# ZhengdiYu/Arbitrary-Hands-3D-Reconstruction

Measured on AMD Instinct MI355X. Metric: frames/sec (2-hand mesh) at 512x512 batch-64; vertex L2 vs ref, higher is better.
Workload: dtype f32; 1 GPU; configs[2]: synthetic 512x512 RGB batch=64 per GPU, HRNet-W32 backbone, fp32; frames_per_gpu=64, global_batch=64, parallelism=frame-sharded x1, gather=none (one rank), contexts_in_turn=2

## Files before the change

### arbitrary-hands-3d-reconstruction_amd/csrc/acrmi.hip

```cpp
#include "acrmi_ctx.h"
#include "score_plan.h"
#include "surface_contact_plan.h"
#include "vertex_color_plan.h"

#include <initializer_list>
#include <type_traits>

std::string g_err;

int fail(acrmi_ctx* c, int code, const char* fmt, ...) {
  char buf[512];
  va_list ap;
  va_start(ap, fmt);
  vsnprintf(buf, sizeof buf, fmt, ap);
  va_end(ap);
  if (c) c->err = buf; else g_err = buf;
  return code;
}

void release_weights(acrmi_ctx* c) {
  if (c->weights_ref && c->weights_ref->fetch_sub(1) == 1) {
    (void)hipFree(c->weights);
    delete c->weights_ref;
  }
// ... 1062 lines not shown
  if (!c->faces_topo[0] || !c->faces_topo[1]) return fail(c, ACRMI_ESTATE, "%s: MANO faces not loaded (acrmi_load_faces)", who);
  ON_DEVICE(c);
  RenderScratch sc;
  if (int r = render_scratch(c, n, &sc)) return r;
  hipError_t e = launch_render_region_prep(slots, offsets, region_frame, n, n_frames, H, W, ACRMI_SLOT, ACRMI_SLOT_FLAG,
                                           colors_host ? colors_host : kHandColors, sc.mesh_frame, sc.mesh_topo, sc.rgb, sc.view,
                                           (hipStream_t)stream);
  if (e != hipSuccess) return fail(c, ACRMI_EHIP, "render region prep: %s", hipGetErrorString(e));
  e = render_launch(c, sc, verts, cam_trans, nullptr, sc.view, focal, visible_weight, img_in, img_out, ids_out, 2 * n, n_frames, H, W,
                    (hipStream_t)stream, vcol);
  return e == hipSuccess ? ACRMI_OK : fail(c, ACRMI_EHIP, "render regions: %s", hipGetErrorString(e));
}

int acrmi_render_regions(acrmi_ctx* c, const float* verts, const float* cam_trans, const float* slots, int n, const float* offsets,
                         const int32_t* region_frame, const float* colors_host, float focal, float visible_weight,
                         const uint8_t* img_in, uint8_t* img_out, int n_frames, int H, int W, int32_t* ids_out, void* stream) {
  return render_regions_call(c, "acrmi_render_regions", false, nullptr, verts, cam_trans, slots, n, offsets, region_frame, colors_host,
                             focal, visible_weight, img_in, img_out, n_frames, H, W, ids_out, stream);
}

int acrmi_render_regions_colored(acrmi_ctx* c, const float* verts, const float* cam_trans, const float* slots, int n,
                                 const float* offsets, const int32_t* region_frame, const float* colors_host, const float* vcol,
                                 float focal, float visible_weight, const uint8_t* img_in, uint8_t* img_out, int n_frames, int H,
                                 int W, int32_t* ids_out, void* stream) {
  return render_regions_call(c, "acrmi_render_regions_colored", true, vcol, verts, cam_trans, slots, n, offsets, region_frame,
                             colors_host, focal, visible_weight, img_in, img_out, n_frames, H, W, ids_out, stream);
}

int acrmi_overlay_regions(acrmi_ctx* c, int what, const float* slots, const float* pj2d_org, int n, const float* offsets,
                          const int32_t* region_frame, int bgr, const uint8_t* img_in, uint8_t* out, uint8_t* out2, int n_frames,
                          int H, int W, void* stream) {
  if (!offsets || !region_frame || n > 0x3fffffff) return fail(c, ACRMI_EINVAL, "acrmi_overlay_regions: bad arguments");
  if (int r = check_overlay(c, "acrmi_overlay_regions", what, slots, pj2d_org, n, img_in, out, out2, n_frames, H, W)) return r;
  ON_DEVICE(c);
  hipError_t e;
  if (what == ACRMI_OVERLAY_SKELETON) {
    if (n > c->region_hand_cap) {
      if (c->region_hand_frame) {
        HIPCHK(c, hipDeviceSynchronize());
        (void)hipFree(c->region_hand_frame);
        c->region_hand_frame = nullptr;
        c->region_hand_cap = 0;
      }
      HIPCHK(c, hipMalloc(&c->region_hand_frame, sizeof(int32_t) * 2 * (size_t)n));
      c->region_hand_cap = n;
    }
    e = launch_render_region_prep(slots, offsets, region_frame, n, n_frames, H, W, ACRMI_SLOT, ACRMI_SLOT_FLAG, nullptr,
                                  c->region_hand_frame, nullptr, nullptr, nullptr, (hipStream_t)stream);
    if (e != hipSuccess) return fail(c, ACRMI_EHIP, "overlay region prep: %s", hipGetErrorString(e));
    e = skeleton_launch(pj2d_org, nullptr, c->region_hand_frame, 0, 2 * n, n_frames, H, W, bgr, img_in, out, (hipStream_t)stream);
  } else {
    RegionHeatmapArgs a{};
    if (int r = heatmap_fill(c, "acrmi_overlay_regions", a, n, offsets, bgr, img_in, out, out2, H, W)) return r;
    a.n_frames = n_frames; a.region_frame = region_frame;
    e = launch_region_heatmap(a, (hipStream_t)stream);
  }
  return e == hipSuccess ? ACRMI_OK : fail(c, ACRMI_EHIP, "overlay regions: %s", hipGetErrorString(e));
}

int acrmi_stream_create(int device, void** stream) {
  if (!stream) return fail(nullptr, ACRMI_EINVAL, "acrmi_stream_create: null argument");
  int prev = 0;
  if (hipGetDevice(&prev) != hipSuccess || hipSetDevice(device) != hipSuccess)
    return fail(nullptr, ACRMI_EHIP, "acrmi_stream_create: cannot select device %d", device);
  hipStream_t st = nullptr;
  const hipError_t e = hipStreamCreateWithFlags(&st, hipStreamNonBlocking);
  (void)hipSetDevice(prev);
  if (e != hipSuccess) return fail(nullptr, ACRMI_EHIP, "hipStreamCreate: %s", hipGetErrorString(e));
  *stream = st;
  return ACRMI_OK;
}

int acrmi_stream_destroy(void* stream) {
  if (!stream) return ACRMI_OK;
  const hipError_t e = hipStreamDestroy((hipStream_t)stream);
  return e == hipSuccess ? ACRMI_OK : fail(nullptr, ACRMI_EHIP, "hipStreamDestroy: %s", hipGetErrorString(e));
}

int acrmi_tune(int key, int value) {
  if (key == 0) { conv_force_cfg(value); return ACRMI_OK; }
  if (key == 3) { conv_set_phase_delay(value); return ACRMI_OK; }
  if (key == 4) { conv_set_xcd_swizzle(value); return ACRMI_OK; }
  if (key == 5) { program_set_grouping(value != 0); return ACRMI_OK; }
  static long long* dbg = nullptr;
  if (key == 1) {
    if (value && !dbg) { if (hipMalloc(&dbg, 128 * sizeof(long long)) != hipSuccess) return ACRMI_EHIP; }
    if (dbg) (void)hipMemset(dbg, 0, 128 * sizeof(long long));
    conv_set_debug(value ? dbg : nullptr);
    return ACRMI_OK;
  }
  if (key == 2) {
    if (!dbg) return ACRMI_OK;
    long long h[128];
    if (hipDeviceSynchronize() != hipSuccess) return ACRMI_EHIP;
    if (hipMemcpy(h, dbg, sizeof h, hipMemcpyDeviceToHost) != hipSuccess) return ACRMI_EHIP;
    const int n = (int)h[63];
    printf("conv stamps (%d):", n);
    for (int i = 1; i < n && i < 60; ++i) printf(" %lld", h[i] - h[i - 1]);
    printf("\n");
    const int nl = (int)h[127];
    if (nl > 0) {
      printf("loader stamps (%d):", nl);
      for (int i = 1; i < nl && i < 60; ++i) printf(" %lld", h[64 + i] - h[64 + i - 1]);
      printf("\n");
    }
    return ACRMI_OK;
  }
  return fail(nullptr, ACRMI_EINVAL, "acrmi_tune: unknown key %d", key);
}

}
```

### arbitrary-hands-3d-reconstruction_amd/csrc/conv_mfma.hip

```cpp
#include "conv_frame.h"
#include "../../include/acrmi.h"
#include <cstdio>
#include <cstdlib>
#include <mutex>

namespace acrmi {

static int g_force_cfg = -1;
void conv_force_cfg(int cfg) { g_force_cfg = cfg; }
static long long* g_dbg = nullptr;
void conv_set_debug(long long* dbg) { g_dbg = dbg; }
static int g_phase_delay = 0;
void conv_set_phase_delay(int cycles) { g_phase_delay = cycles; }
static int g_xcd_swizzle = 1;
void conv_set_xcd_swizzle(int on) { g_xcd_swizzle = on; }
static int g_num_cus_dev[MAX_DEVICES] = {};
template <int KS, int S, int TH, int TW, int CK, int NLW>
__device__ __forceinline__ void dma_loader(const ConvArgs& a, const ConvWork& wk, float* lds, int ltid, int my_items,
                                           int nchunks, int vb) {
  constexpr int PH = (TH - 1) * S + KS, PW = (TW - 1) * S + KS, CP = CK + 4, PAD = KS / 2, BUF = PH * PW * CP;
  constexpr int SPP = CK / 4 + 1;
  constexpr int NSLOT = PH * PW * SPP, NI = (NSLOT + NLW * 64 - 1) / (NLW * 64);
  const int lane = ltid & 63;
  const int lw = __builtin_amdgcn_readfirstlane(ltid >> 6);
// ... 368 lines not shown
}

static long pick_grid(long total) {
  const long grid = g_num_cus_dev[current_device()];
  return grid > total ? total : grid;
}

int conv_forced_cfg() { return g_force_cfg; }
int conv_num_cus() { return g_num_cus_dev[current_device()]; }
hipError_t conv_ensure_device_info() { return ensure_device_info(); }

static hipError_t conv_first_use(const void* fn, unsigned char* flags, const ConvKernel& k, const char* form, int threads, size_t lds) {
  if (!first_use_on_device(flags)) return hipSuccess;
  hipError_t e = hipFuncSetAttribute(fn, hipFuncAttributeMaxDynamicSharedMemorySize, (int)lds);
  if (e != hipSuccess) return e;
  if (getenv("ACRMI_DEBUG")) {
    hipFuncAttributes fa;
    (void)hipFuncGetAttributes(&fa, fn);
    fprintf(stderr, "[acrmi] %s%s in %s: threads %d lds %zu regs %d scratch %zu\n", k.name, form, k.where, threads, lds, fa.numRegs,
            (size_t)fa.localSizeBytes);
  }
  return hipSuccess;
}
static bool conv_work(ConvWork& wk, int tiles_x, int tiles_y, int nblk, int nb_inner, const ConvArgs& a) {
  wk.tiles_x = tiles_x;
  wk.tiles_per_frame = tiles_x * tiles_y;
  wk.n_tiles_total = wk.tiles_per_frame * a.B;
  wk.nblk = nblk;
  wk.nb_inner = nb_inner;
  wk.total = wk.n_tiles_total * wk.nblk * a.groups;
  if ((unsigned long long)wk.total * (unsigned long long)wk.n_tiles_total >= (1ull << 40)) return false;
  set_magics(wk);
  return true;
}

hipError_t launch_conv_kernel(const ConvKernel& k, int threads, size_t lds, int tiles_x, int tiles_y, int nblk,
                              const ConvArgs& a, hipStream_t s, int nb_inner) {
  hipError_t e = conv_first_use(reinterpret_cast<const void*>(k.fn), k.first_use, k, "", threads, lds);
  if (e != hipSuccess) return e;
  ConvWork wk;
  if (!conv_work(wk, tiles_x, tiles_y, nblk, nb_inner, a)) return hipErrorInvalidValue;
  hipLaunchKernelGGL(k.fn, dim3((unsigned)pick_grid(wk.total)), dim3(threads), lds, s, a, wk);
  return hipGetLastError();
}

hipError_t launch_conv_kernel(const ConvKernel& k, int threads, size_t lds, const ConvProblem* p, int n, hipStream_t s) {
  if (!p || n < 1 || n > CONV_GROUP_MAX) return hipErrorInvalidValue;
  if (n == 1) return launch_conv_kernel(k, threads, lds, p[0].tiles_x, p[0].tiles_y, p[0].nblk, p[0].a, s);
  if (!k.group_fn) return hipErrorInvalidValue;
  hipError_t e = conv_first_use(reinterpret_cast<const void*>(k.group_fn), k.group_first_use, k, " (group form)", threads, lds);
  if (e != hipSuccess) return e;
  ConvGroup g;
  long total = 0;
  for (int i = 0; i < n; ++i) {
    g.a[i] = p[i].a;
    if (!conv_work(g.wk[i], p[i].tiles_x, p[i].tiles_y, p[i].nblk, 1, p[i].a) || g.wk[i].total <= 0) return hipErrorInvalidValue;
    total += g.wk[i].total;
  }
  if (total >= (1l << 30)) return hipErrorInvalidValue;
  hipLaunchKernelGGL(k.group_fn, dim3((unsigned)pick_grid(total)), dim3(threads), lds, s, g);
  return hipGetLastError();
}

template <int TH, int TW, int WAVES_M, int WAVES_N, int CK, int NLW>
static hipError_t launch_wino(const ConvArgs& a, hipStream_t s) {
  constexpr size_t lds = 2 * (size_t)(TH + 2) * (TW + 2) * (CK + 4) * sizeof(float) +
                         2 * (size_t)(WAVES_M * WAVES_N) * 2 * 1024 * sizeof(float);
  static_assert(lds <= 160 * 1024, "patch and residual buffers must fit the 160 KiB LDS");
  return launch_conv_kernel(CONV_KERNEL(conv_wino_kernel<TH, TW, WAVES_M, WAVES_N, CK, NLW>), (WAVES_M * WAVES_N + NLW) * 64, lds,
                            (a.Wo + TW - 1) / TW, (a.Ho + TH - 1) / TH, (a.n_tiles + WAVES_N - 1) / WAVES_N, a, s);
}

#include "conv_wino2.inc"
#include "conv_ws2.inc"
#include "conv_wino3.inc"
#include "conv_wino24.inc"
#include "conv_wino24b.inc"
#include "conv_wino24c.inc"
#include "conv_pp2.inc"
#include "conv_x3.inc"
#include "conv_x3p.inc"
#include "conv_x3s2.inc"
#include "conv_p1.inc"

static hipError_t conv_prepare(ConvArgs& a) {
  a.dbg = g_dbg;
  a.phase_delay = g_phase_delay;
  static const char* swz_env = experiment_env("ACRMI_XCD_SWIZZLE");
  a.xcd_swizzle = swz_env ? atoi(swz_env) : g_xcd_swizzle;
  {
    static float* zeros[MAX_DEVICES] = {};
    const int dev = current_device();
    std::lock_guard<std::recursive_mutex> lock(g_init_mutex);
    if (!zeros[dev]) {
      float* z = nullptr;
      hipError_t e = hipMalloc(&z, 256);
      if (e != hipSuccess) return e;
      if ((e = hipMemset(z, 0, 256)) != hipSuccess || (e = hipDeviceSynchronize()) != hipSuccess) {
        (void)hipFree(z);
        return e;
      }
      zeros[dev] = z;
    }
    a.zeros = zeros[dev];
  }
  return ensure_device_info();
}

static const void* conv_group_instance(const ConvArgs& a, int* tw_out) {
  if (a.dtype != ACRMI_DT_F32 || a.algo != 4 || conv_algo_reject(a.algo, conv_shape(a)) || wino24c_ok(a)) return nullptr;
  const int tw = wino24b_ok(a);
  Wino24bPick p;
  if (!tw || !wino24b_pick(a, tw, p) || !p.k.group_fn) return nullptr;
  if (tw_out) *tw_out = tw;
  return reinterpret_cast<const void*>(p.k.fn);
}
bool conv_can_group(const ConvArgs& a, const ConvArgs& b) {
  const void* ka = conv_group_instance(a, nullptr);
  return ka && ka == conv_group_instance(b, nullptr);
}

hipError_t launch_conv_group(const ConvArgs* a, int n, hipStream_t s) {
  if (!a || n < 1 || n > CONV_GROUP_MAX) return hipErrorInvalidValue;
  if (n == 1) return launch_conv(a[0], s);
  std::lock_guard<std::recursive_mutex> launch_lock(g_init_mutex);
  ConvArgs p[CONV_GROUP_MAX];
  int tw[CONV_GROUP_MAX];
  for (int i = 0; i < n; ++i) {
    p[i] = a[i];
    hipError_t e = conv_prepare(p[i]);
    if (e != hipSuccess) return e;
    if (!conv_group_instance(p[i], &tw[i]) || !conv_can_group(p[0], p[i])) return hipErrorInvalidValue;
  }
  return launch_wino24b_group(p, tw, n, s);
}

hipError_t launch_conv(ConvArgs a, hipStream_t s) {
  if (conv_algo_reject(a.algo, conv_shape(a))) return hipErrorInvalidValue;
  std::lock_guard<std::recursive_mutex> launch_lock(g_init_mutex);
  {
    hipError_t de = conv_prepare(a);
    if (de != hipSuccess) return de;
  }
  if (a.dtype != ACRMI_DT_F32) return launch_conv_h16(a, s);
  const bool n32 = a.n_tiles == 1;
  const bool small = (a.Ho * a.Wo <= 256) || (a.Ho % 16 != 0) || (a.Wo % 16 != 0);
  if ((a.algo == 6 || a.algo == 7) && a.ks == 1) return launch_x3p(a, a.algo == 7, s);
  if ((a.algo == 6 || a.algo == 7) && a.stride == 2) return launch_x3s2(a, a.algo == 7, s);
  if (a.algo == 6 || a.algo == 7) return launch_x3(a, a.algo == 7, s);
  if (a.algo == 5) return launch_pp2(a, s);
  if (a.algo == 4)
    {
      if (wino24c_ok(a)) return launch_wino24c(a, s);
      const int tw = wino24b_ok(a);
      return tw ? launch_wino24b(a, tw, s) : launch_wino24(a, s);
    }
  if (a.algo == 3) return launch_wino3(a, s);
  if (a.algo == 2) {
    if (a.splitk) return launch_wino2<1, 32, 2>(a, s);
    const bool odd33 = a.Cout == 33 && a.groups == 1 && a.cin8 * 8 > 32 && g_force_cfg != 804;
    const long items2 = (long)((a.Ho + 7) / 8) * ((a.Wo + 15) / 16) * a.B * ((a.n_tiles + 1) / 2) * a.groups;
    const bool few = items2 < g_num_cus_dev[current_device()] && g_force_cfg != 806;
    const bool nt1 = n32 || a.cin8 * 8 <= 32 || odd33 || few;
    if (!n32 && !odd33 && !few && a.cin8 == 2 && g_force_cfg != 807) return launch_wino2<2, 8, 2>(a, s);
    if (g_force_cfg == 801) return nt1 ? launch_wino2<1, 32, 4>(a, s) : launch_wino2<2, 32, 4>(a, s);
    return nt1 ? launch_wino2<1, 32, 2>(a, s) : launch_wino2<2, 32, 2>(a, s);
  }
  if (a.algo == 1) {
    if (n32) return small ? launch_wino<8, 16, 2, 1, 32, 2>(a, s) : launch_wino<16, 16, 4, 1, 32, 2>(a, s);
    return launch_wino<8, 16, 2, 2, 32, 2>(a, s);
  }
  if (a.nxt > 0)
    return launch_ws2_impl<3, 2, 8, 16, 4, 1, 1, 1, 16, 2, false, true>(a, s);
  if (a.ks == 3 && a.stride == 1) {
    if (n32) return small ? launch_ws2<3, 1, 8, 16, 4, 1, 1, 1, 32, 2>(a, s) : launch_ws2<3, 1, 16, 16, 4, 2, 1, 1, 32, 2>(a, s);
    return small ? launch_ws2<3, 1, 8, 16, 2, 2, 2, 1, 32, 2>(a, s) : launch_ws2<3, 1, 16, 16, 4, 2, 1, 2, 32, 2>(a, s);
  }
  const long cus = g_num_cus_dev[current_device()];
  const long tiles8 = (long)((a.Ho + 7) / 8) * ((a.Wo + 15) / 16) * a.B * a.groups;
  const long tiles16 = (long)((a.Ho + 15) / 16) * ((a.Wo + 15) / 16) * a.B * a.groups;
  const int nb2 = (a.n_tiles + 1) / 2;
  const bool fine = g_force_cfg != 806;
  if (a.ks == 3 && a.stride == 2) {
    if (n32 || (fine && tiles8 * nb2 < cus)) return launch_ws2<3, 2, 8, 16, 4, 1, 1, 1, 16, 2>(a, s);
    return launch_ws2<3, 2, 8, 16, 2, 2, 2, 1, 16, 2>(a, s);
  }
  if (a.ks == 1 && a.stride == 2) {
    ConvArgs b = a;
    b.stride = 1;
    b.in_sub = 2;
    return launch_conv(b, s);
  }
  if (a.ks == 1 && a.stride == 1) {
    if (p1_ok(a) && g_force_cfg != 809 &&
        (long)((a.Ho * a.Wo) / 256) * a.B * a.groups * ((a.Cout / 32) / (a.Cout % 64 == 0 ? 2 : 1)) >= 2 * cus)
      return launch_p1(a, s);
    if (n32) return (small || (fine && tiles16 < cus)) ? launch_ws2<1, 1, 8, 16, 4, 1, 1, 1, 64, 2>(a, s)
                                                        : launch_ws2<1, 1, 16, 16, 4, 2, 1, 1, 64, 4>(a, s);
    if ((fine && (tiles8 * nb2 < cus || (a.Cin <= 64 && tiles8 * nb2 <= 4 * cus))) || g_force_cfg == 808)
      return launch_ws2<1, 1, 8, 16, 4, 1, 1, 1, 64, 2>(a, s);
    return (small || (fine && tiles16 * nb2 < cus)) ? launch_ws2<1, 1, 8, 16, 2, 2, 2, 1, 64, 2>(a, s)
                                                    : launch_ws2<1, 1, 16, 16, 4, 2, 1, 2, 64, 4>(a, s);
  }
  return hipErrorInvalidValue;
}

const char* conv_kernel_name(const ConvArgs& a) {
  if (a.dtype != ACRMI_DT_F32) return a.dtype == ACRMI_DT_BF16 ? "conv_direct_mfma_bf16" : "conv_direct_mfma_f16";
  if (a.algo == 7) return a.ks == 1 ? "conv1x1_split_bf16x3_mfma" : (a.stride == 2 ? "conv3x3s2_split_bf16x3_mfma" : "conv3x3s1_split_bf16x3_mfma");
  if (a.algo == 6) return a.ks == 1 ? "conv1x1_split_f16x3_mfma" : (a.stride == 2 ? "conv3x3s2_split_f16x3_mfma" : "conv3x3s1_split_f16x3_mfma");
  if (a.algo == 5) return "conv3x3s2_polyphase_mfma_f32";
  if (a.algo == 4) return "conv3x3s1_wino2x4_mfma_f32";
  if (a.algo == 3) return "conv3x3s1_wino2d_lds_mfma_f32";
  if (a.algo == 2) return "conv3x3s1_wino2d_mfma_f32";
  if (a.algo == 1) return "conv3x3s1_wino_mfma_f32";
  if (a.ks == 3 && a.stride == 1) return "conv3x3s1_mfma_f32";
  if (a.ks == 3 && a.stride == 2) return "conv3x3s2_mfma_f32";
  return "conv1x1_mfma_f32";
}

}
```

### arbitrary-hands-3d-reconstruction_amd/csrc/conv_rules.h

```cpp
#pragma once

namespace acrmi {

struct ConvShape {
  int ks, stride, groups, cin, cout, H, W, Ho, Wo;
  int in_cs, in_coff, out_cs, out_coff, res_cs, res_coff, out2_cs, out2_coff;
  int has_res;
  int bias_fstride;
  int nxt, out2;
  int splitk, res_bcast, in_sub;
  int dtype, out_f32;
};

constexpr int conv_out_size(int in, int ks, int stride) { return (in + 2 * (ks / 2) - ks) / stride + 1; }
constexpr int conv_n_tiles(int cout) { return cout <= 32 ? 1 : ((cout + 63) / 64) * 2; }
constexpr int conv_ksteps(int cin, int dtype) { return dtype ? (cin + 15) / 16 : (cin + 7) / 8; }
constexpr int conv_taps(int algo, int ks) { return algo >= 6 ? ks * ks : algo == 5 ? 28 : algo == 4 ? 24 : algo >= 2 ? 16 : algo == 1 ? 12 : ks * ks; }
constexpr long long conv_weight_floats(int algo, int groups, int ks, int cin, int cout, int dtype) {
  return algo == 3 ? 16384 : (long long)groups * conv_taps(algo, ks) * conv_ksteps(cin, dtype) * conv_n_tiles(cout) * 256 + (algo >= 6);
}

inline bool conv_in_aligned(const ConvShape& s) { return s.in_cs % 4 == 0 && s.in_coff % 4 == 0; }
inline bool conv_out_aligned(const ConvShape& s) { return s.out_cs % 4 == 0 && s.out_coff % 4 == 0; }
inline bool conv_res_aligned(const ConvShape& s) { return !s.has_res || (s.res_cs % 4 == 0 && s.res_coff % 4 == 0); }
inline bool conv_c32(const ConvShape& s) { return s.cin % 32 == 0 && s.cin >= 32 && s.cout % 32 == 0; }
inline bool conv_same_map(const ConvShape& s) { return s.H == s.Ho && s.W == s.Wo; }
inline bool conv_frame4(const ConvShape& s, int halo_rows) {
  return conv_in_aligned(s) && conv_out_aligned(s) && conv_res_aligned(s) && !s.splitk && s.in_sub <= 1 &&
         (halo_rows ? (long long)halo_rows * s.W : 256) * s.in_cs * 4 < (1ll << 30) &&
         (s.bias_fstride == 0 || s.bias_fstride >= s.groups * conv_n_tiles(s.cout) * 32);
}

inline bool takes_wino3(const ConvShape& s) {
  return s.ks == 3 && s.stride == 1 && s.groups == 1 && s.cin <= 32 && s.cout == 32 && s.bias_fstride == 0 && s.Ho % 8 == 0 &&
         s.Wo % 16 == 0 && conv_out_aligned(s) && conv_in_aligned(s) && conv_res_aligned(s);
}
inline int takes_wino24b(const ConvShape& s) {
  if (!(s.ks == 3 && s.stride == 1 && conv_c32(s) && conv_same_map(s) && conv_frame4(s, 10))) return 0;
  if (s.Ho % 8 == 0 && s.Wo % 32 == 0) return 32;
  return (s.Ho % 16 == 0 && s.Wo % 16 == 0 && s.cout % 64 == 0 && s.cin >= 64) ? 16 : 0;
}
inline bool takes_wino24c(const ConvShape& s) { return takes_wino24b(s) == 32 && s.cin >= 64 && s.cout % 64 == 0; }
inline bool takes_pp2(const ConvShape& s) {
  return s.ks == 3 && s.stride == 2 && s.H % 2 == 0 && s.W % 2 == 0 && s.Ho == s.H / 2 && s.Wo == s.W / 2 && s.Ho % 8 == 0 &&
         s.Wo % 16 == 0 && s.cin % 16 == 0 && s.cout % 32 == 0 && conv_frame4(s, 17);
}
inline int takes_x3(const ConvShape& s) {
  if (!(s.ks == 3 && s.stride == 1 && conv_c32(s) && conv_same_map(s) && conv_frame4(s, 18))) return 0;
  return (s.Ho % 8 == 0 && s.Wo % 32 == 0) ? 32 : (s.Ho % 16 == 0 && s.Wo % 16 == 0) ? 16 : 0;
}
inline bool takes_x3s2(const ConvShape& s) {
  return s.ks == 3 && s.stride == 2 && conv_c32(s) && s.H == 2 * s.Ho && s.W == 2 * s.Wo && s.Ho % 8 == 0 && s.Wo % 32 == 0 &&
         s.nxt == 0 && conv_frame4(s, 34);
}
inline bool takes_p1(const ConvShape& s) {
  return s.ks == 1 && s.stride == 1 && conv_c32(s) && conv_same_map(s) && (s.Ho * s.Wo) % 256 == 0 && conv_frame4(s, 0);
}
inline bool takes_x3p(const ConvShape& s) { return takes_p1(s); }
inline bool takes_dma(const ConvShape& s) { return s.cin % 4 == 0 && conv_in_aligned(s); }

inline const char* conv_algo_reject(int algo, const ConvShape& s) {
  if (algo < 0 || algo > 7) return "unknown conv algo (0..7)";
  if ((s.ks != 1 && s.ks != 3) || (s.stride != 1 && s.stride != 2)) return "only 3x3 and 1x1 convolutions at stride 1 / 2 are implemented";
  if (s.nxt < 0 || s.nxt > 3) return "at most 3 extra residual terms";
  if (s.dtype) {
    if (algo != 0 || s.splitk || s.nxt || s.out2 || s.res_bcast)
      return "16-bit storage runs the direct kernels only: algo 0, no split-K, extra residual terms, second output or bias map";
    if (s.out_f32 && s.stride != 1) return "16-bit input with fp32 output exists at stride 1 only";
    const int oq = s.out_f32 ? 4 : 8;
    return (s.in_cs % 8 || s.in_coff % 8 || (s.groups > 1 && s.cin % 8) || s.out_cs % oq || (s.has_res && s.res_cs % oq))
               ? "16-bit storage: channel strides, the input offset and a group's first channel must be multiples of 16 bytes" : nullptr;
  }
  if (!conv_in_aligned(s) || (s.groups > 1 && s.cin % 4)) return "in_cs, in_coff and a group's first channel must be multiples of 4";
  if (s.splitk && (algo != 2 || s.groups < 2 || s.groups > 8 || s.cin % 32 || s.cin < 64 || s.cout == 33 || s.bias_fstride))
    return "split-K needs algo 2, 2..8 slices of Cin % 32 == 0, Cin >= 64 channels each, Cout != 33, no per-frame bias";
  if (s.nxt > 0 && algo != 5 && algo != 0 && !(algo == 3 && s.out2))
    return "extra residual terms need a 3x3 stride-2 convolution (algo 0 / 5) or the second output of algo 3";
  if (s.out2 && algo != 3) return "a second output needs algo 3";
  if (s.res_bcast && algo == 3) return "a position-bias map needs an algo other than 3";
  auto why = [&](int halo_rows, const char* geometry) {
    return conv_frame4(s, halo_rows) ? geometry : "the four-wave frame needs in_cs, in_coff, out_cs, out_coff, res_cs, res_coff % 4 == 0, a per-frame "
                                                  "bias row of groups * n_tiles * 32 floats, a halo patch below 2^30 bytes";
  };
  const bool s11 = s.ks == 3 && s.stride == 1;
  if (algo >= 6 && s.ks == 1) return takes_x3p(s) ? nullptr : why(0, "algo 6 / 7 (1x1) needs stride 1, Cin % 32 == 0, Cout % 32 == 0, a map of whole 256-pixel items");
  if (algo >= 6 && s.stride == 2)
    return takes_x3s2(s) ? nullptr : why(34, "algo 6 / 7 at stride 2 needs Cin % 32 == 0, Cout % 32 == 0, an even input size (H = 2 Ho, W = 2 Wo), an output map of "
                                             "8x32-pixel tiles, no extra residual terms");
  if (algo >= 6) return takes_x3(s) ? nullptr : why(18, "algo 6 / 7 (3x3 stride 1) needs Cin % 32 == 0, Cout % 32 == 0, a map of 8x32- or 16x16-pixel tiles");
  if (algo == 5) return takes_pp2(s) ? nullptr : why(17, "algo 5 needs a 3x3 stride-2 convolution, Cin % 16 == 0, Cout % 32 == 0, an even input size, an output map of 8x16-pixel tiles");
  if (algo == 4)
    return (s11 && (takes_wino24b(s) || conv_ksteps(s.cin, 0) * 8 > 32)) ? nullptr
           : "algo 4 needs a 3x3 stride-1 convolution with Cin > 32 - or Cin = 32 with Cout % 32 == 0 on a map of 8x32-pixel tiles, 16-byte aligned channel slices";
  if (algo == 3 && !takes_wino3(s))
    return "algo 3 needs a 3x3 stride-1 convolution, groups 1, Cin <= 32, Cout = 32, no per-frame bias, a map of 8x16-pixel tiles, out_cs, out_coff, res_cs, res_coff % 4 == 0";
  if (algo == 3 && s.out2 && (!takes_dma(s) || s.nxt < 1 || s.out2_cs % 4 || s.out2_coff % 4))
    return "the second output of algo 3 needs Cin % 4 == 0, 1..3 extra residual terms, out2_cs, out2_coff % 4 == 0";
  if ((algo == 1 || algo == 2) && !s11) return "algo 1 / 2 needs a 3x3 stride-1 convolution";
  if (algo == 0 && s.nxt > 0 && (s.ks != 3 || s.stride != 2 || conv_ksteps(s.cin, 0) * 8 <= 16 || s.cout % 32 || !conv_out_aligned(s)))
    return "extra residual terms on algo 0 need a 3x3 stride-2 convolution with Cin > 16, Cout % 32 == 0, out_cs, out_coff % 4 == 0";
  return nullptr;
}

}
```

### arbitrary-hands-3d-reconstruction_amd/csrc/heads.hip

```cpp
#include "kernels.h"
#include "../../include/acrmi.h"

namespace acrmi {

typedef float f32x16 __attribute__((ext_vector_type(16)));
typedef float f32x4 __attribute__((ext_vector_type(4)));

constexpr int ATT_SCHUNKS = 64;
constexpr int ATT_KSPLIT = 32;

__global__ __launch_bounds__(256) void att_stats_kernel(const float* __restrict__ segm, int segm_cs, int H, int W,
                                                        float* __restrict__ ws) {
  const int b = blockIdx.x, chunk = blockIdx.y;
  const int part = threadIdx.x & 31, grp = threadIdx.x >> 5;
  const int npix = H * W, per = npix / ATT_SCHUNKS;
  const float* base = segm + (size_t)b * (2 * H) * (2 * W) * segm_cs + 1 + part;
  float m = -INFINITY, s = 0.f;
  for (int q = chunk * per + grp; q < (chunk + 1) * per; q += 32) {
    float v[4];
#pragma unroll
    for (int u = 0; u < 4; ++u) {
      const int qq = q + 8 * u, y = qq / W, x = qq % W;
      v[u] = base[((size_t)(2 * y) * (2 * W) + 2 * x) * segm_cs];
    }
#pragma unroll
    for (int u = 0; u < 4; ++u) {
      const float nm = fmaxf(m, v[u]);
      s = s * expf(m - nm) + expf(v[u] - nm);
      m = nm;
    }
  }
  __shared__ float sm[8][32], ss[8][32];
  sm[grp][part] = m;
  ss[grp][part] = s;
  __syncthreads();
  if (threadIdx.x < 32) {
    float M = sm[0][part];
    for (int g = 1; g < 8; ++g) M = fmaxf(M, sm[g][part]);
    float S = 0.f;
    for (int g = 0; g < 8; ++g) S += ss[g][part] * expf(sm[g][part] - M);
    float* o = ws + (((size_t)b * ATT_SCHUNKS + chunk) * 32 + part) * 2;
    o[0] = M;
    o[1] = S;
  }
}

template <int NTILES, int FDT = 0>
__global__ __launch_bounds__(256) void att_pool_kernel(const float* __restrict__ segm, int segm_cs,
                                                       const float* __restrict__ feat, int feat_cs, int H, int W,
                                                       const float* __restrict__ stats, float* __restrict__ part_ws) {
  const int b = blockIdx.x, ks = blockIdx.y;
  const int lane = threadIdx.x & 63, wave = threadIdx.x >> 6;
  const int li = lane & 31, lh = lane >> 5;
  float M = -INFINITY;
  {
    const float* st = stats + ((size_t)b * ATT_SCHUNKS * 32 + li) * 2;
#pragma unroll 8
    for (int c = 0; c < ATT_SCHUNKS; ++c) M = fmaxf(M, st[(size_t)c * 64]);
  }
  const int npix = H * W;
  const int per_wave = npix / (ATT_KSPLIT * 4);
  const int q0 = (ks * 4 + wave) * per_wave;
  const float* sbase = segm + (size_t)b * (2 * H) * (2 * W) * segm_cs + 1 + li;
  const float* fbase = feat + (size_t)b * npix * feat_cs + li;
  const unsigned short* hbase = reinterpret_cast<const unsigned short*>(feat) + (size_t)b * npix * feat_cs + li;
  f32x16 acc[NTILES];
#pragma unroll
  for (int n = 0; n < NTILES; ++n)
#pragma unroll
    for (int r = 0; r < 16; ++r) acc[n][r] = 0.f;
  constexpr int U = NTILES > 8 ? 2 : 4;
  for (int q = q0 + lh; q < q0 + per_wave; q += 2 * U) {
    float lv[U], bv[U][NTILES];
#pragma unroll
    for (int u = 0; u < U; ++u) {
      const int qq = q + 2 * u, y = qq / W, x = qq % W;
      lv[u] = sbase[((size_t)(2 * y) * (2 * W) + 2 * x) * segm_cs];
      if constexpr (FDT == 0) {
        const float* f = fbase + (size_t)qq * feat_cs;
#pragma unroll
        for (int n = 0; n < NTILES; ++n) bv[u][n] = f[n * 32];
      } else {
        const unsigned short* f = hbase + (size_t)qq * feat_cs;
#pragma unroll
        for (int n = 0; n < NTILES; ++n) {
          if constexpr (FDT == 2) bv[u][n] = (float)__builtin_bit_cast(__bf16, f[n * 32]);
          else bv[u][n] = (float)__builtin_bit_cast(_Float16, f[n * 32]);
        }
      }
    }
#pragma unroll
    for (int u = 0; u < U; ++u) {
      const float a = expf(lv[u] - M);
#pragma unroll
      for (int n = 0; n < NTILES; ++n) acc[n] = __builtin_amdgcn_mfma_f32_32x32x2f32(a, bv[u][n], acc[n], 0, 0, 0);
    }
  }
  constexpr int NH = NTILES < 4 ? NTILES : 4;
  __shared__ float red[4][NH * 1024];
  float* o = part_ws + (size_t)(b * ATT_KSPLIT + ks) * 32 * (NTILES * 32);
  for (int n0 = 0; n0 < NTILES; n0 += NH) {
#pragma unroll
    for (int n = 0; n < NTILES; ++n)
      if (n >= n0 && n < n0 + NH) {
#pragma unroll
        for (int r = 0; r < 16; ++r) red[wave][(n - n0) * 1024 + r * 64 + lane] = acc[n][r];
      }
    __syncthreads();
    const int cnt = (NTILES - n0 < NH ? NTILES - n0 : NH) * 1024;
    for (int idx = threadIdx.x; idx < cnt; idx += 256) {
      const float sum = ((red[0][idx] + red[1][idx]) + red[2][idx]) + red[3][idx];
      const int n = n0 + (idx >> 10), r = (idx >> 6) & 15, l = idx & 63;
      const int p = (r & 3) + 8 * (r >> 2) + 4 * (l >> 5);
      o[(size_t)p * (NTILES * 32) + n * 32 + (l & 31)] = sum;
    }
    __syncthreads();
  }
}

__global__ __launch_bounds__(256) void att_reduce_kernel(const float* __restrict__ part_ws,
                                                         const float* __restrict__ stats, int C,
                                                         float* __restrict__ pooled) {
  const int b = blockIdx.x;
  __shared__ float inv[32];
  if (threadIdx.x < 32) {
    const int p = threadIdx.x;
    float M = -INFINITY;
    for (int c = 0; c < ATT_SCHUNKS; ++c) M = fmaxf(M, stats[(((size_t)b * ATT_SCHUNKS + c) * 32 + p) * 2]);
    float S = 0.f;
    for (int c = 0; c < ATT_SCHUNKS; ++c) {
      const float* st = stats + (((size_t)b * ATT_SCHUNKS + c) * 32 + p) * 2;
      S += st[1] * expf(st[0] - M);
    }
    inv[p] = 1.f / S;
  }
  __syncthreads();
  const int n = 32 * C;
  const int i = blockIdx.y * 256 + threadIdx.x;
  const float* src = part_ws + (size_t)b * ATT_KSPLIT * n + i;
  float s = 0.f;
  for (int k = 0; k < ATT_KSPLIT; k += 8) {
    float t[8];
#pragma unroll
    for (int u = 0; u < 8; ++u) t[u] = src[(size_t)(k + u) * n];
#pragma unroll
    for (int u = 0; u < 8; ++u) s += t[u];
  }
  pooled[(size_t)b * n + i] = s * inv[i / C];
}

size_t attpool_ws_floats(int B, int C) {
  return (size_t)B * ATT_SCHUNKS * 32 * 2 + (size_t)B * ATT_KSPLIT * 32 * C;
}

hipError_t launch_attpool(const float* segm, int segm_cs, const float* feat, int feat_cs, int C, int B, int H, int W,
                          float* ws, float* pooled, hipStream_t s, int feat_dtype) {
  const int npix = H * W;
  if (npix % (ATT_KSPLIT * 4 * 8) != 0 || npix % (ATT_SCHUNKS * 32) != 0 || (32 * C) % 256 != 0) return hipErrorInvalidValue;
  float* stats_ws = ws;
  float* part_ws = ws + (size_t)B * ATT_SCHUNKS * 32 * 2;
  hipLaunchKernelGGL(att_stats_kernel, dim3(B, ATT_SCHUNKS), dim3(256), 0, s, segm, segm_cs, H, W, stats_ws);
  if (feat_dtype != 0) {
    if (C != 256 || feat_dtype < 0 || feat_dtype > 2) return hipErrorInvalidValue;
    if (feat_dtype == 2)
      hipLaunchKernelGGL((att_pool_kernel<8, 2>), dim3(B, ATT_KSPLIT), dim3(256), 0, s, segm, segm_cs, feat, feat_cs, H, W,
                         stats_ws, part_ws);
    else
      hipLaunchKernelGGL((att_pool_kernel<8, 1>), dim3(B, ATT_KSPLIT), dim3(256), 0, s, segm, segm_cs, feat, feat_cs, H, W,
                         stats_ws, part_ws);
  } else if (C == 320)
    hipLaunchKernelGGL(att_pool_kernel<10>, dim3(B, ATT_KSPLIT), dim3(256), 0, s, segm, segm_cs, feat, feat_cs, H, W,
                       stats_ws, part_ws);
  else if (C == 256)
    hipLaunchKernelGGL(att_pool_kernel<8>, dim3(B, ATT_KSPLIT), dim3(256), 0, s, segm, segm_cs, feat, feat_cs, H, W,
                       stats_ws, part_ws);
  else if (C == 64)
    hipLaunchKernelGGL(att_pool_kernel<2>, dim3(B, ATT_KSPLIT), dim3(256), 0, s, segm, segm_cs, feat, feat_cs, H, W,
                       stats_ws, part_ws);
  else if (C == 32)
    hipLaunchKernelGGL(att_pool_kernel<1>, dim3(B, ATT_KSPLIT), dim3(256), 0, s, segm, segm_cs, feat, feat_cs, H, W,
                       stats_ws, part_ws);
  else
    return hipErrorInvalidValue;
  hipLaunchKernelGGL(att_reduce_kernel, dim3(B, 32 * C / 256), dim3(256), 0, s, part_ws, stats_ws, C, pooled);
  return hipGetLastError();
}

__global__ __launch_bounds__(256) void parebias_kernel(const PareArgs a) {
  const int b = blockIdx.x, tid = threadIdx.x;
  __shared__ float pl[16 * 320];
  const int shape_c0 = a.C == 320 ? 256 : 0, shape_n = (a.C - shape_c0) * 16;
  __shared__ float pare[112];
  __shared__ float red[10][4];
  for (int i = tid; i < 16 * a.C; i += 256) pl[i] = a.pooled[((size_t)b * 32 + a.part0) * a.C + i];
  __syncthreads();
  if (tid < 96) {
    const int j = tid / 6, o = tid % 6;
    float s = 0.f;
    for (int c = 0; c < 256; ++c) s += a.lc_w[(o * 256 + c) * 16 + j] * pl[j * a.C + c];
    pare[tid] = s;
  }
  float part[10];
#pragma unroll
  for (int k = 0; k < 10; ++k) part[k] = 0.f;
  for (int i = tid; i < shape_n; i += 256) {
    const float x = pl[(i & 15) * a.C + shape_c0 + (i >> 4)];
#pragma unroll
    for (int k = 0; k < 10; ++k) part[k] += a.lin_w[k * shape_n + i] * x;
  }
#pragma unroll
  for (int k = 0; k < 10; ++k) {
    float v = part[k];
    for (int off = 32; off > 0; off >>= 1) v += __shfl_down(v, off, 64);
    if ((tid & 63) == 0) red[k][tid >> 6] = v;
  }
  __syncthreads();
  if (tid < 10) pare[96 + tid] = a.lin_b[tid] + ((red[tid][0] + red[tid][1]) + (red[tid][2] + red[tid][3]));
  __syncthreads();
  if (tid < 109) {
    float s = a.mix_b[tid];
    for (int k = 0; k < 106; ++k) s += a.mix_wp[tid * 106 + k] * pare[k];
    a.out[(size_t)b * a.out_stride + tid] = s;
  } else if (tid < a.out_stride) {
    a.out[(size_t)b * a.out_stride + tid] = 0.f;
  }
}
hipError_t launch_parebias(const PareArgs& a, hipStream_t s) {
  if ((a.C != 320 && a.C != 256) || a.out_stride > 256) return hipErrorInvalidValue;
  hipLaunchKernelGGL(parebias_kernel, dim3(a.B), dim3(256), 0, s, a);
  return hipGetLastError();
}

__device__ inline void rotmat_t_to_aa(const float* t, float* aa) {
  const float t00 = t[0], t01 = t[1], t02 = t[2];
  const float t10 = t[3], t11 = t[4], t12 = t[5];
  const float t20 = t[6], t21 = t[7], t22 = t[8];
  float q[4], tr;
  if (t22 < 1e-6f) {
    if (t00 > t11) {
      tr = 1.f + t00 - t11 - t22;
      q[0] = t12 - t21; q[1] = tr; q[2] = t01 + t10; q[3] = t20 + t02;
    } else {
      tr = 1.f - t00 + t11 - t22;
      q[0] = t20 - t02; q[1] = t01 + t10; q[2] = tr; q[3] = t12 + t21;
    }
  } else {
    if (t00 < -t11) {
      tr = 1.f - t00 - t11 + t22;
      q[0] = t01 - t10; q[1] = t20 + t02; q[2] = t12 + t21; q[3] = tr;
    } else {
      tr = 1.f + t00 + t11 + t22;
      q[0] = tr; q[1] = t12 - t21; q[2] = t20 - t02; q[3] = t01 - t10;
    }
  }
// ... 735 lines not shown
```

### arbitrary-hands-3d-reconstruction_amd/csrc/kernels.h

```cpp
#pragma once
#include <hip/hip_runtime.h>
#include <stdint.h>
#include <mutex>

#include <stdlib.h>

#include "conv_rules.h"
#include "nv12_out_plan.h"
#include "smooth_plan.h"
#include "assoc_plan.h"
#include "point_plan.h"

namespace acrmi {

inline const char* experiment_env(const char* name) {
#ifdef ACRMI_EXPERIMENTS
  return getenv(name);
#else
  (void)name;
  return nullptr;
#endif
}

struct ConvArgs {
  const float* in;
  const float* w;
  const float* bias;
  const float* res;
  float* out;
  int B, H, W, Ho, Wo;
  int in_cs, in_coff, Cin;
  int out_cs, out_coff, Cout;
  int res_cs, res_coff;
  int ks, stride, relu, groups;
  int n_tiles;
  int cin8;
  int bias_fstride;
  int algo;
  long long* dbg;
  int phase_delay;
  int xcd_swizzle;
  const float* zeros;
  int dtype;
  int out_f32;
  int res_bcast;
  int in_sub;
  int splitk;
  float* split_ws;
  unsigned* split_cnt;
  int nxt;
  const float* xt[3];
  int xt_cs[3], xt_coff[3], xt_shift[3];
  float* out2;
  int out2_cs, out2_coff;
  unsigned* range_flag;
};
inline void conv_derive(ConvArgs& a) {
  a.Ho = conv_out_size(a.H, a.ks, a.stride);
  a.Wo = conv_out_size(a.W, a.ks, a.stride);
  a.cin8 = conv_ksteps(a.Cin, a.dtype);
  a.n_tiles = conv_n_tiles(a.Cout);
}
inline size_t conv_splitk_groups(int B, int Ho, int Wo, int cout) {
  return (size_t)B * ((Ho + 7) / 8) * ((Wo + 15) / 16) * conv_n_tiles(cout);
}
inline size_t conv_splitk_ws_floats(int B, int Ho, int Wo, int cout, int splits) { return conv_splitk_groups(B, Ho, Wo, cout) * splits * 4096; }
inline size_t conv_splitk_counters(int B, int Ho, int Wo, int cout) { return conv_splitk_groups(B, Ho, Wo, cout) * 4; }

constexpr int MAX_DEVICES = 64;
bool first_use_on_device(unsigned char* flags);
std::recursive_mutex& launch_mutex();

hipError_t launch_conv(ConvArgs a, hipStream_t s);
hipError_t launch_conv_h16(ConvArgs a, hipStream_t s);
bool conv_can_group(const ConvArgs& a, const ConvArgs& b);
hipError_t launch_conv_group(const ConvArgs* a, int n, hipStream_t s);
const char* conv_kernel_name(const ConvArgs& a);
void conv_force_cfg(int cfg);
void conv_set_debug(long long* dbg);
void conv_set_phase_delay(int cycles);
void conv_set_xcd_swizzle(int on);

hipError_t launch_u8norm(const uint8_t* img, long n_pixels, float* out, hipStream_t s);
bool stem_shape_ok(int H, int W, int out_cs, int out_coff);
hipError_t launch_stem(const uint8_t* img, int B, int H, int W, const float* wpk, const float* bias, float* out,
                       int out_cs, int out_coff, int relu, hipStream_t s);
hipError_t launch_pair1x1(const float* t2, int t2_cs, int t2_coff, const float* x, int x_cs, int x_coff, float* y, int y_cs,
                          int y_coff, float* t, int t_cs, int t_coff, const float* wpk, long npix, hipStream_t s);
constexpr long PAIR1X1_FLOATS = 256 * 64 + 64 * 256 + 256 + 64;
bool stem7_shape_ok(int H, int W, int out_cs, int out_coff);
hipError_t launch_stem7(const uint8_t* img, int B, int H, int W, const float* wpk, const float* bias, float* out,
                        int out_cs, int out_coff, int relu, hipStream_t s);
hipError_t launch_stem7_h16(const uint8_t* img, int B, int H, int W, const float* wpk, const float* bias, void* out,
                            int out_cs, int out_coff, int relu, int dtype, hipStream_t s);
hipError_t launch_stem_h16(const uint8_t* img, int B, int H, int W, const float* wpk, const float* bias, void* out,
                           int out_cs, int out_coff, int relu, int dtype, hipStream_t s);
hipError_t launch_bilinear2x(const float* in, int B, int H, int W, int in_cs, int in_coff, int C, float* out,
                             int out_cs, int out_coff, hipStream_t s);
struct FuseArgs {
  const float* term[4];
  int cs[4], shift[4];
  int nterms, B, H, W, C, out_cs, relu;
  float* out;
};
hipError_t launch_fuse_sum(const FuseArgs& a, hipStream_t s);
__device__ inline void cv_cubic_taps(int d, double scale, int& s0, int (&c)[4]) {
  float f = (float)(((double)d + 0.5) * scale - 0.5);
  const float fl = floorf(f);
  s0 = (int)fl;
  f -= fl;
  const float A = -0.75f;
  float k[4];
  k[0] = ((A * (f + 1.f) - 5.f * A) * (f + 1.f) + 8.f * A) * (f + 1.f) - 4.f * A;
  k[1] = ((A + 2.f) * f - (A + 3.f)) * f * f + 1.f;
  k[2] = ((A + 2.f) * (1.f - f) - (A + 3.f)) * (1.f - f) * (1.f - f) + 1.f;
  k[3] = 1.f - k[0] - k[1] - k[2];
#pragma unroll
  for (int i = 0; i < 4; ++i) {
    int v = (int)rintf(k[i] * 2048.f);
    c[i] = v < -32768 ? -32768 : (v > 32767 ? 32767 : v);
  }
}
hipError_t launch_preprocess(const uint8_t* bgr, int n, int H, int W, int out_size, uint8_t* out, hipStream_t s);
constexpr int NV12_FRAMES_PER_LAUNCH = 64;
struct Nv12Coef {
  int cy, cub, cug, cvg, cvr, y_off;
};
struct Nv12DstFrame {
  const uint8_t* y;
  const uint8_t* uv;
  uint8_t* dst;
  int H, W, y_pitch, uv_pitch;
};
struct Nv12DstBatch {
  Nv12DstFrame f[NV12_FRAMES_PER_LAUNCH];
};
static_assert(sizeof(Nv12DstBatch) + sizeof(Nv12Coef) + 8 <= 4096, "NV12 kernel arguments must fit the 4 KB argument block");
hipError_t launch_nv12_to_rgb(const Nv12DstBatch& pb, const Nv12Coef& k, int n, int bgr, hipStream_t s);
__device__ inline int nv12_clamp8(int v) { return v < 0 ? 0 : (v > 255 ? 255 : v); }
__device__ inline void nv12_pixel(const Nv12Coef& k, int Y, int U, int V, int& R, int& G, int& B) {
  int yy = Y - k.y_off;
  yy = (yy < 0 ? 0 : yy) * k.cy;
  const int u = U - 128, v = V - 128, r = 1 << 19;
  R = nv12_clamp8((yy + k.cvr * v + r) >> 20);
  G = nv12_clamp8((yy + k.cug * u + k.cvg * v + r) >> 20);
  B = nv12_clamp8((yy + k.cub * u + r) >> 20);
}
struct Nv12OutFrame {
  const uint8_t* src;
  uint8_t* y;
  uint8_t* uv;
  int H, W, y_pitch, uv_pitch;
};
struct Nv12OutBatch {
  Nv12OutFrame f[NV12_FRAMES_PER_LAUNCH];
};
constexpr int NV12_COMPOSE_FRAMES_PER_LAUNCH = 58;
struct Nv12ComposeFrame {
  const uint8_t* src_y;
  const uint8_t* src_uv;
  const uint8_t* drawn;
// ... 361 lines not shown
```

Measured before the change: 2023 frames/s.

## Add register-pipelined 1x1 conv kernel and float4 attention-pool path

Adds a new 1x1 stride-1 fp32 MFMA conv kernel (q1). It streams activations and weights straight from global memory into an 8-deep register ring, with no LDS staging. It is chosen when the existing ws2 paths would launch fewer than about two work items per CU. Separately, the 256-channel attention pooling gets a variant that loads two float4 per lane with an 8-deep prefetch ring and a remapped reduction. Both aim to hide memory latency on low-occupancy layers, at the cost of more register pressure and more dispatch heuristics.

```diff
diff --git a/arbitrary-hands-3d-reconstruction_amd/csrc/acrmi.hip b/arbitrary-hands-3d-reconstruction_amd/csrc/acrmi.hip
--- a/arbitrary-hands-3d-reconstruction_amd/csrc/acrmi.hip
+++ b/arbitrary-hands-3d-reconstruction_amd/csrc/acrmi.hip
@@ -1168,6 +1168,7 @@
   if (key == 3) { conv_set_phase_delay(value); return ACRMI_OK; }
   if (key == 4) { conv_set_xcd_swizzle(value); return ACRMI_OK; }
   if (key == 5) { program_set_grouping(value != 0); return ACRMI_OK; }
+  if (key == 6) return (int)(conv_q1_launches() & 0x7fffffff);
   static long long* dbg = nullptr;
   if (key == 1) {
     if (value && !dbg) { if (hipMalloc(&dbg, 128 * sizeof(long long)) != hipSuccess) return ACRMI_EHIP; }
diff --git a/arbitrary-hands-3d-reconstruction_amd/csrc/conv_mfma.hip b/arbitrary-hands-3d-reconstruction_amd/csrc/conv_mfma.hip
--- a/arbitrary-hands-3d-reconstruction_amd/csrc/conv_mfma.hip
+++ b/arbitrary-hands-3d-reconstruction_amd/csrc/conv_mfma.hip
@@ -474,6 +474,7 @@
 #include "conv_x3p.inc"
 #include "conv_x3s2.inc"
 #include "conv_p1.inc"
+#include "conv_q1.inc"
 
 static hipError_t conv_prepare(ConvArgs& a) {
   a.dbg = g_dbg;
@@ -587,6 +588,19 @@
     if (p1_ok(a) && g_force_cfg != 809 &&
         (long)((a.Ho * a.Wo) / 256) * a.B * a.groups * ((a.Cout / 32) / (a.Cout % 64 == 0 ? 2 : 1)) >= 2 * cus)
       return launch_p1(a, s);
+    if (q1_ok(a) && g_force_cfg != 810) {
+      const bool one = a.cin8 * 8 <= 64 && g_force_cfg != 901;
+      const bool thin = (fine && (tiles8 * nb2 < cus || (a.Cin <= 64 && tiles8 * nb2 <= 4 * cus))) || g_force_cfg == 808;
+      long items;
+      if (n32) items = (small || (fine && tiles16 < cus)) ? tiles8 : tiles16;
+      else if (thin) items = tiles8 * (one ? 1 : a.n_tiles);
+      else {
+        const bool t8 = small || (fine && tiles16 * nb2 < cus);
+        items = (t8 ? tiles8 : tiles16) * (one ? 1 : nb2);
+        if (!t8 && items >= cus) items = 2 * cus;
+      }
+      if (items < 2 * cus) return launch_q1(a, s);
+    }
     if (n32) return (small || (fine && tiles16 < cus)) ? launch_ws2<1, 1, 8, 16, 4, 1, 1, 1, 64, 2>(a, s)
                                                         : launch_ws2<1, 1, 16, 16, 4, 2, 1, 1, 64, 4>(a, s);
     if ((fine && (tiles8 * nb2 < cus || (a.Cin <= 64 && tiles8 * nb2 <= 4 * cus))) || g_force_cfg == 808)
diff --git a/arbitrary-hands-3d-reconstruction_amd/csrc/conv_q1.inc b/arbitrary-hands-3d-reconstruction_amd/csrc/conv_q1.inc
--- /dev/null
+++ b/arbitrary-hands-3d-reconstruction_amd/csrc/conv_q1.inc
@@ -0,0 +1,104 @@
+
+template <int NT, int WG>
+__global__ __launch_bounds__(WG * 64) void conv_q1_kernel(const ConvArgs a, const int ptiles, const int nblk) {
+  constexpr int R = 8;
+  const int lane = threadIdx.x & 63;
+  const int wave = __builtin_amdgcn_readfirstlane((int)threadIdx.x >> 6);
+  const int li = lane & 31, lh = lane >> 5;
+  const int bx = (int)blockIdx.x, r8 = bx >> 3;
+  const int nb = r8 % nblk;
+  const int ptile = ((r8 / nblk) * 8 + (bx & 7)) * WG + wave;
+  if (ptile >= ptiles) return;
+  const int nt0 = nb * NT;
+  const int nsteps = a.cin8;
+
+  const float* __restrict__ xin = a.in + a.in_coff + ((size_t)ptile * 32 + li) * a.in_cs + 4 * lh;
+  const __amdgpu_buffer_rsrc_t wrsrc =
+      __builtin_amdgcn_make_buffer_rsrc(const_cast<float*>(a.w), 0, a.cin8 * a.n_tiles * 1024, 0x00020000);
+  const int step_b = a.n_tiles * 1024;
+  const unsigned wlane = lane * 16;
+  f32x4 act[R], wgt[R][NT];
+  auto load = [&](int r, int step) {
+    const int sc = step < nsteps ? step : nsteps - 1;
+    act[r] = *reinterpret_cast<const f32x4*>(xin + sc * 8);
+#pragma unroll
+    for (int n = 0; n < NT; ++n)
+      wgt[r][n] = __builtin_bit_cast(f32x4, __builtin_amdgcn_raw_buffer_load_b128(wrsrc, wlane, sc * step_b + (nt0 + n) * 1024, 0));
+  };
+  f32x16 acc[NT];
+#pragma unroll
+  for (int n = 0; n < NT; ++n)
+#pragma unroll
+    for (int i = 0; i < 16; ++i) acc[n][i] = 0.f;
+#pragma unroll
+  for (int u = 0; u < R; ++u) {
+    load(u, u);
+    __builtin_amdgcn_sched_barrier(0);
+  }
+  int s = 0;
+  for (; s + R <= nsteps; s += R) {
+#pragma unroll
+    for (int u = 0; u < R; ++u) {
+      __builtin_amdgcn_sched_barrier(0);
+#pragma unroll
+      for (int j = 0; j < 4; ++j)
+#pragma unroll
+        for (int n = 0; n < NT; ++n) acc[n] = __builtin_amdgcn_mfma_f32_32x32x2f32(wgt[u][n][j], act[u][j], acc[n], 0, 0, 0);
+      __builtin_amdgcn_sched_barrier(0);
+      load(u, s + u + R);
+    }
+    __builtin_amdgcn_sched_barrier(0);
+  }
+  for (; s < nsteps; ++s) {
+    load(0, s);
+#pragma unroll
+    for (int j = 0; j < 4; ++j)
+#pragma unroll
+      for (int n = 0; n < NT; ++n) acc[n] = __builtin_amdgcn_mfma_f32_32x32x2f32(wgt[0][n][j], act[0][j], acc[n], 0, 0, 0);
+  }
+  const size_t pix = (size_t)ptile * 32 + li;
+  float* __restrict__ outp = a.out + a.out_coff + pix * a.out_cs + 4 * lh;
+  const float* __restrict__ resp = a.res ? a.res + a.res_coff + pix * a.res_cs + 4 * lh : nullptr;
+#pragma unroll
+  for (int n = 0; n < NT; ++n) {
+    const int co = (nt0 + n) * 32;
+    f32x4 bv[4], rv[4];
+#pragma unroll
+    for (int q = 0; q < 4; ++q) {
+      bv[q] = *reinterpret_cast<const f32x4*>(a.bias + co + 8 * q + 4 * lh);
+      rv[q] = resp ? __builtin_nontemporal_load(reinterpret_cast<const f32x4*>(resp + co + 8 * q)) : f32x4{0.f, 0.f, 0.f, 0.f};
+    }
+#pragma unroll
+    for (int q = 0; q < 4; ++q) {
+      f32x4 o4 = f32x4{acc[n][4 * q], acc[n][4 * q + 1], acc[n][4 * q + 2], acc[n][4 * q + 3]} + bv[q] + rv[q];
+      if (a.relu) {
+        o4[0] = vrelu1(o4[0]); o4[1] = vrelu1(o4[1]); o4[2] = vrelu1(o4[2]); o4[3] = vrelu1(o4[3]);
+      }
+      *reinterpret_cast<f32x4*>(outp + co + 8 * q) = o4;
+    }
+  }
+}
+
+static bool q1_ok(const ConvArgs& a) { return a.algo == 0 && takes_q1(conv_shape(a)); }
+static long g_q1_launches = 0;
+long conv_q1_launches() { return g_q1_launches; }
+
+template <int NT, int WG>
+static hipError_t launch_q1_impl(const ConvArgs& a, hipStream_t s) {
+  const long ptiles = (long)a.B * a.Ho * a.Wo / 32;
+  const int nblk = (a.Cout / 32) / NT;
+  const long blocks = ((ptiles + WG - 1) / WG + 7) / 8 * 8 * nblk;
+  if (ptiles >= (1l << 26) || blocks >= (1l << 31)) return hipErrorInvalidValue;
+  hipLaunchKernelGGL((conv_q1_kernel<NT, WG>), dim3((unsigned)blocks), dim3(WG * 64), 0, s, a, (int)ptiles, nblk);
+  ++g_q1_launches;
+  return hipGetLastError();
+}
+static hipError_t launch_q1(const ConvArgs& a, hipStream_t s) {
+  const long cus = g_num_cus_dev[current_device()];
+  const long waves2 = (long)a.B * a.Ho * a.Wo / 32 * (a.Cout / 64);
+  const bool n2 = a.Cout % 64 == 0 && (waves2 >= 4 * cus || g_force_cfg == 816) && g_force_cfg != 815;
+  const int wg = g_force_cfg == 813 ? 2 : g_force_cfg == 814 ? 4 : 1;
+  if (wg == 4) return n2 ? launch_q1_impl<2, 4>(a, s) : launch_q1_impl<1, 4>(a, s);
+  if (wg == 2) return n2 ? launch_q1_impl<2, 2>(a, s) : launch_q1_impl<1, 2>(a, s);
+  return n2 ? launch_q1_impl<2, 1>(a, s) : launch_q1_impl<1, 1>(a, s);
+}
diff --git a/arbitrary-hands-3d-reconstruction_amd/csrc/conv_rules.h b/arbitrary-hands-3d-reconstruction_amd/csrc/conv_rules.h
--- a/arbitrary-hands-3d-reconstruction_amd/csrc/conv_rules.h
+++ b/arbitrary-hands-3d-reconstruction_amd/csrc/conv_rules.h
@@ -57,6 +57,11 @@
   return s.ks == 1 && s.stride == 1 && conv_c32(s) && conv_same_map(s) && (s.Ho * s.Wo) % 256 == 0 && conv_frame4(s, 0);
 }
 inline bool takes_x3p(const ConvShape& s) { return takes_p1(s); }
+inline bool takes_q1(const ConvShape& s) {
+  return s.dtype == 0 && s.ks == 1 && s.stride == 1 && s.groups == 1 && s.in_sub <= 1 && !s.splitk && s.nxt == 0 && !s.out2 &&
+         s.bias_fstride == 0 && !s.res_bcast && s.cin % 8 == 0 && s.cin >= 8 && s.cout % 32 == 0 && s.cout >= 32 && conv_same_map(s) &&
+         (s.Ho * s.Wo) % 32 == 0 && conv_in_aligned(s) && conv_out_aligned(s) && conv_res_aligned(s);
+}
 inline bool takes_dma(const ConvShape& s) { return s.cin % 4 == 0 && conv_in_aligned(s); }
 
 inline const char* conv_algo_reject(int algo, const ConvShape& s) {
diff --git a/arbitrary-hands-3d-reconstruction_amd/csrc/heads.hip b/arbitrary-hands-3d-reconstruction_amd/csrc/heads.hip
--- a/arbitrary-hands-3d-reconstruction_amd/csrc/heads.hip
+++ b/arbitrary-hands-3d-reconstruction_amd/csrc/heads.hip
@@ -6,6 +6,7 @@
 typedef float f32x16 __attribute__((ext_vector_type(16)));
 typedef float f32x4 __attribute__((ext_vector_type(4)));
 
+int conv_forced_cfg();
 constexpr int ATT_SCHUNKS = 64;
 constexpr int ATT_KSPLIT = 32;
 
@@ -45,7 +46,7 @@
   }
 }
 
-template <int NTILES, int FDT = 0>
+template <int NTILES, int FDT = 0, bool X4 = false>
 __global__ __launch_bounds__(256) void att_pool_kernel(const float* __restrict__ segm, int segm_cs,
                                                        const float* __restrict__ feat, int feat_cs, int H, int W,
                                                        const float* __restrict__ stats, float* __restrict__ part_ws) {
@@ -69,6 +70,37 @@
   for (int n = 0; n < NTILES; ++n)
 #pragma unroll
     for (int r = 0; r < 16; ++r) acc[n][r] = 0.f;
+  if constexpr (X4) {
+    static_assert(NTILES == 8 && FDT == 0, "two float4 per lane = 256 fp32 channels");
+    constexpr int R = 8;
+    const int ntrips = per_wave / 2;
+    float lv[R];
+    f32x4 fv[R][2];
+    auto load = [&](int r, int t) {
+      const int qq = q0 + 2 * (t < ntrips ? t : ntrips - 1) + lh, y = qq / W, x = qq % W;
+      lv[r] = sbase[((size_t)(2 * y) * (2 * W) + 2 * x) * segm_cs];
+      const f32x4* f = reinterpret_cast<const f32x4*>(fbase + (size_t)qq * feat_cs + 3 * li);
+      fv[r][0] = f[0];
+      fv[r][1] = f[32];
+    };
+#pragma unroll
+    for (int u = 0; u < R; ++u) {
+      load(u, u);
+      __builtin_amdgcn_sched_barrier(0);
+    }
+    for (int t = 0; t < ntrips; t += R) {
+#pragma unroll
+      for (int u = 0; u < R; ++u) {
+        __builtin_amdgcn_sched_barrier(0);
+        const float a = expf(lv[u] - M);
+#pragma unroll
+        for (int n = 0; n < NTILES; ++n) acc[n] = __builtin_amdgcn_mfma_f32_32x32x2f32(a, fv[u][n >> 2][n & 3], acc[n], 0, 0, 0);
+        __builtin_amdgcn_sched_barrier(0);
+        load(u, t + u + R);
+      }
+      __builtin_amdgcn_sched_barrier(0);
+    }
+  } else {
   constexpr int U = NTILES > 8 ? 2 : 4;
   for (int q = q0 + lh; q < q0 + per_wave; q += 2 * U) {
     float lv[U], bv[U][NTILES];
@@ -96,6 +128,7 @@
       for (int n = 0; n < NTILES; ++n) acc[n] = __builtin_amdgcn_mfma_f32_32x32x2f32(a, bv[u][n], acc[n], 0, 0, 0);
     }
   }
+  }
   constexpr int NH = NTILES < 4 ? NTILES : 4;
   __shared__ float red[4][NH * 1024];
   float* o = part_ws + (size_t)(b * ATT_KSPLIT + ks) * 32 * (NTILES * 32);
@@ -109,10 +142,12 @@
     __syncthreads();
     const int cnt = (NTILES - n0 < NH ? NTILES - n0 : NH) * 1024;
     for (int idx = threadIdx.x; idx < cnt; idx += 256) {
-      const float sum = ((red[0][idx] + red[1][idx]) + red[2][idx]) + red[3][idx];
-      const int n = n0 + (idx >> 10), r = (idx >> 6) & 15, l = idx & 63;
+      const int ri = X4 ? (idx & 3) * 1024 + (idx >> 8) * 64 + ((idx >> 2) & 63) : idx;
+      const float sum = ((red[0][ri] + red[1][ri]) + red[2][ri]) + red[3][ri];
+      const int n = n0 + (ri >> 10), r = (ri >> 6) & 15, l = ri & 63;
       const int p = (r & 3) + 8 * (r >> 2) + 4 * (l >> 5);
-      o[(size_t)p * (NTILES * 32) + n * 32 + (l & 31)] = sum;
+      const int ch = X4 ? 128 * (n >> 2) + 4 * (l & 31) + (n & 3) : n * 32 + (l & 31);
+      o[(size_t)p * (NTILES * 32) + ch] = sum;
     }
     __syncthreads();
   }
@@ -170,6 +205,9 @@
                          stats_ws, part_ws);
   } else if (C == 320)
     hipLaunchKernelGGL(att_pool_kernel<10>, dim3(B, ATT_KSPLIT), dim3(256), 0, s, segm, segm_cs, feat, feat_cs, H, W,
+                       stats_ws, part_ws);
+  else if (C == 256 && conv_forced_cfg() != 811 && feat_cs % 4 == 0 && ((size_t)feat & 15) == 0 && npix % (ATT_KSPLIT * 4 * 16) == 0)
+    hipLaunchKernelGGL((att_pool_kernel<8, 0, true>), dim3(B, ATT_KSPLIT), dim3(256), 0, s, segm, segm_cs, feat, feat_cs, H, W,
                        stats_ws, part_ws);
   else if (C == 256)
     hipLaunchKernelGGL(att_pool_kernel<8>, dim3(B, ATT_KSPLIT), dim3(256), 0, s, segm, segm_cs, feat, feat_cs, H, W,
diff --git a/arbitrary-hands-3d-reconstruction_amd/csrc/kernels.h b/arbitrary-hands-3d-reconstruction_amd/csrc/kernels.h
--- a/arbitrary-hands-3d-reconstruction_amd/csrc/kernels.h
+++ b/arbitrary-hands-3d-reconstruction_amd/csrc/kernels.h
@@ -77,6 +77,7 @@
 hipError_t launch_conv_group(const ConvArgs* a, int n, hipStream_t s);
 const char* conv_kernel_name(const ConvArgs& a);
 void conv_force_cfg(int cfg);
+long conv_q1_launches();
 void conv_set_debug(long long* dbg);
 void conv_set_phase_delay(int cycles);
 void conv_set_xcd_swizzle(int on);
```

Result: no change. 2025 frames/s (median of 5 runs) (+0.1%).
